# fraunhoferhhi/vvenc

Measured on AMD Instinct MI355X. Metric: frames/sec + bit-exact vs CPU, 1080p/4K 10-bit preset=faster at 1/2/4/8 GPU, higher is better.
Workload: dtype i16; 1 GPU; BASELINE configs[1]: hot-path work lists RECORDED from the reference encoder (1920x1080 10-bit synthetic clip, 65 frames, preset faster; one picture per temporal layer), replayed resident in HBM: a step = one picture's integer-ME SAD windows + sub-pel SATD stages + table calls + fused TU transform/quant lists + DMVR lists on 5 HIP streams; steps follow the GOP's 1:1:2:4:8:16 layer mix from the key; hip_streams=5, sample_pairs_per_frame=175309451, coefficients_per_frame=6951461, recorded_calls_outside_the_lists=0

## Files before the change

### vvenc_amd/csrc/trquant.hip

```cpp
#include "common.h"
#include <stdlib.h>
#include <string.h>
#include <algorithm>
#include <vector>

namespace {

typedef uint32_t u32x2 __attribute__( ( ext_vector_type( 2 ) ) );
typedef uint32_t u32x4 __attribute__( ( ext_vector_type( 4 ) ) );
typedef short    s16x2 __attribute__( ( ext_vector_type( 2 ) ) );

__device__ __forceinline__ int clip3i( int lo, int hi, int v ) { return v < lo ? lo : ( v > hi ? hi : v ); }
__device__ __forceinline__ int sat16( int v ) { return clip3i( -32768, 32767, v ); }
__device__ __forceinline__ int dot2( uint32_t a, uint32_t b, int acc )
{
  return __builtin_amdgcn_sdot2( __builtin_bit_cast( s16x2, a ), __builtin_bit_cast( s16x2, b ), acc, false );
}

struct TrGeom
{
  int w, h, log2w, log2h;
  int skipW, skipH;
  int shift1, shift2;
};
// ... 919 lines not shown
      }
    }
  };
  uint32_t xr[8];
  loadResidual( waveIndex, xr );

  const int rndF1 = A.shF1 > 0 ? 1 << ( A.shF1 - 1 ) : 0, rndF2 = 1 << ( A.shF2 - 1 ), rndI1 = 1 << ( A.shI1 - 1 ), rndI2 = 1 << ( A.shI2 - 1 );
  const bool liveCol = inL < N - A.skipW, liveRow = mxSigma( c32 ) % N < N - A.skipH;
  const v4i zero4 = { 0, 0, 0, 0 };
  sOps[lane]       = liveCol ? *reinterpret_cast<const v4i*>( A.opH->nat[lane] ) : zero4;
  sOps[64 + lane]  = liveRow ? *reinterpret_cast<const v4i*>( A.opV->rowP[lane] ) : zero4;
  const int cP1 = ( liveCol ? A.opH->rowSum[c32] : 0 ) + rndF1, cI1 = A.opV->colSum[c32] + rndI1;
  sInit[c32]      = ( c32 % N < N - A.skipH ? A.opV->rowSum[c32] : 0 ) + rndF2;
  sInit[32 + c32] = A.opH->colSum[c32] + rndI2;
  uint32_t pos[16];
  {
    const u32x4 p0 = *reinterpret_cast<const u32x4*>( A.pos + lane * 16 ), p1 = *reinterpret_cast<const u32x4*>( A.pos + lane * 16 + 8 );
    const uint32_t pw[8] = { p0.x, p0.y, p0.z, p0.w, p1.x, p1.y, p1.z, p1.w };
#pragma unroll
    for( int v = 0; v < 16; v++ ) pos[v] = ( v & 1 ) ? pw[v >> 1] >> 16 : pw[v >> 1] & 0xffffu;
  }
  WAVE_SYNC();
  if( ( A.phaseLimit & 0xff ) == 1 ) return;

  for( int tile = waveIndex; tile < A.tiles; tile += A.waveStride )
  {
    v4i aLo, aHi;
    if( tile != waveIndex ) loadResidual( tile, xr );
#pragma unroll
    for( int g = 0; g < 4; g++ )
    {
      aLo[g] = ( int ) ( __builtin_amdgcn_perm( xr[2 * g + 1], xr[2 * g], 0x06040200u ) ^ 0x80808080u );
      aHi[g] = ( int ) __builtin_amdgcn_perm( xr[2 * g + 1], xr[2 * g], 0x07050301u );
    }
    vvhip_tu_qp qqs[R];
#pragma unroll
    for( int r = 0; r < R; r++ ) { const int tu = tile * TPT + ( blk0 + r ) * TPS + blkL; qqs[r] = tu < A.n ? A.qps[tu] : vvhip_tu_qp{ 32, 0 }; }
    if( ( A.phaseLimit & 0xff ) == 2 ) { int k_ = 0; _Pragma( "unroll" ) for( int g = 0; g < 4; g++ ) k_ ^= aLo[g] ^ aHi[g]; if( k_ == 0x12345678 ) A.stats[0].pad = 1; continue; }

    int d[16];
    v4i bLo, bHi;
    {
      v16i c;
#pragma unroll
      for( int v = 0; v < 16; v++ ) c[v] = cP1;
      const v4i opP1 = sOps[lane];
      MX_PASS( aHi, opP1, aLo, opP1, c, A.shF1 );
      mxSplitSat( d, bLo, bHi );
    }
    {
      v16i c;
#pragma unroll
      for( int g = 0; g < 4; g++ ) { const v4i t = *reinterpret_cast<const v4i*>( &sInit[h * 16 + 4 * g] ); c[4 * g] = t.x; c[4 * g + 1] = t.y; c[4 * g + 2] = t.z; c[4 * g + 3] = t.w; }
      const v4i opP2 = sOps[64 + lane];
      MX_PASS( opP2, bHi, opP2, bLo, c, A.shF2 );
    }
    if( ( A.phaseLimit & 0xff ) == 3 ) { TUMX_KEEP( d ); continue; }

    uint32_t last[R], need[R], big[R];
    bool wide = false, someLevel = false;
#pragma unroll
    for( int r = 0; r < R; r++ )
    {
      const TuMxQ P = tuMxParams( A.q, qqs[r], A.thrVal );
      uint32_t l = 0, mx = 0, bg = 0;
      const int thr4 = P.thres >> 2;
// ... 79 lines not shown
        if( PS == 8 ) { u32x4 v; v.x = rp[0]; v.y = rp[1 % ( PS / 2 )]; v.z = rp[2 % ( PS / 2 )]; v.w = rp[3 % ( PS / 2 )]; *reinterpret_cast<u32x4*>( dst ) = v; } \
        else          { u32x2 v; v.x = rp[0]; v.y = rp[1 % ( PS / 2 )]; *reinterpret_cast<u32x2*>( dst ) = v; } \
      } \
    } \
_Pragma( "unroll" ) \
    for( int r = 0; r < R; r++ ) \
    { \
      const unsigned long long t = vvhipGroupSum64( smallDiff ? ( unsigned long long ) sse32[r] : sse[r], G, lane ); \
      const int tu = tile * TPT + blkL * TPS + blk0 + r; \
      if( A.stats && ( N < 32 || h == 0 ) && inL == r && tu < A.n ) A.stats[tu].sse = t; \
    } }
    const bool allZero = ( N >= TUMX_ZERO_MIN_N ) && __builtin_amdgcn_ballot_w64( someLevel ) == 0ull;
    uint32_t xr2[8];
#define TUMX_REREAD() { _Pragma( "unroll" ) for( int c = 0; c < NP; c++ )                                                                \
      {                                                                                                                                 \
        const int X0 = 16 * h + PS * c;                                                                                                 \
        const int tu = tile * TPT + blkL * TPS + X0 / N;                                                                                \
        const int16_t* src = resi + ( tu < A.n ? A.resiOff[tu] : 0 ) + ( ptrdiff_t ) inL * resiStride + X0 % N;                         \
        if( PS == 8 )                                                                                                                   \
        {                                                                                                                               \
          u32x4 v = { 0, 0, 0, 0 };                                                                                                     \
          if( tu < A.n ) v = reinterpret_cast<const U16*>( src )->v;                                                                    \
          xr2[4 * c] = v.x; xr2[( 4 * c + 1 ) & 7] = v.y; xr2[( 4 * c + 2 ) & 7] = v.z; xr2[( 4 * c + 3 ) & 7] = v.w;                   \
        }                                                                                                                               \
        else                                                                                                                            \
        {                                                                                                                               \
          u32x2 v = { 0, 0 };                                                                                                           \
          if( tu < A.n ) v = reinterpret_cast<const U8*>( src )->v;                                                                     \
          xr2[( 2 * c ) & 7] = v.x; xr2[( 2 * c + 1 ) & 7] = v.y;                                                                       \
        }                                                                                                                               \
      } }
    if( allZero )
    {
#if TUMX_ZERO_KEEP_RESI
#pragma unroll
      for( int k = 0; k < 8; k++ ) xr2[k] = xr[k];
#else
      TUMX_REREAD()
#endif
#pragma unroll
      for( int r = 0; r < R; r++ )
      {
        const int tu = tile * TPT + ( blk0 + r ) * TPS + blkL;
        if( A.stats && ( N < 32 || h == 0 ) && inL == r && tu < A.n )
        {
          int32_t* st = reinterpret_cast<int32_t*>( A.stats + tu );
          st[0] = 0; st[1] = ( int32_t ) last[r]; st[2] = ( int32_t ) need[r]; st[3] = 0;
        }
      }
      if( !( A.phaseLimit & 0x100 ) )
#pragma unroll
      for( int u = 0; u < 16 / PS; u++ )
      {
        const int q = lane + 64 * u, Y = q / ( 32 / PS ), X = PS * ( q % ( 32 / PS ) );
        const int tu = tile * TPT + ( Y / N ) * TPS + X / N;
        if( tu < A.n )
        {
          const size_t at = ( size_t ) tu * N * N + ( Y % N ) * N + X % N;
          if( PS == 8 ) { if( A.level ) *reinterpret_cast<u32x4*>( A.level + at ) = u32x4{ 0, 0, 0, 0 }; if( A.rec ) *reinterpret_cast<u32x4*>( A.rec + at ) = u32x4{ 0, 0, 0, 0 }; }
          else          { if( A.level ) *reinterpret_cast<u32x2*>( A.level + at ) = u32x2{ 0, 0 }; if( A.rec ) *reinterpret_cast<u32x2*>( A.rec + at ) = u32x2{ 0, 0 }; }
        }
      }
#pragma unroll
      for( int v = 0; v < 16; v++ ) d[v] = 0;
      TUMX_TAIL( false )
      continue;
    }
    uint32_t absSum[R];
#define TUMX_LEVELS( MEXPR )                                                                                                           \
    _Pragma( "unroll" ) for( int r = 0; r < R; r++ )                                                                                   \
    {                                                                                                                                  \
      const TuMxQ P = tuMxParams( A.q, qqs[r], A.thrVal );                                                                             \
      uint32_t sum = 0;                                                                                                                \
      const int rsPos = P.rightShift > 0 ? P.rightShift : 0, rndDq = P.rightShift > 0 ? 1 << ( P.rightShift - 1 ) : 0;                \
      const int iscaleL = P.rightShift < 0 ? P.iscale << ( -P.rightShift ) : P.iscale;                                                 \
      _Pragma( "unroll" ) for( int v = r * VPR; v < ( r + 1 ) * VPR; v++ )                                                             \
      {                                                                                                                                \
        const int cv = d[v];                                                                                                           \
        const uint32_t ac = ( uint32_t ) abs( cv );                                                                                    \
        uint32_t m = MEXPR;                                                                                                            \
        m = pos[v] <= last[r] ? m : 0u;                                                                                                \
        sum += m;                                                                                                                      \
        const int sm = cv < 0 ? -( int32_t ) m : ( int32_t ) m;                                                                        \
        const int lv = clip3i( -32768, 32767, sm );                                                                                    \
        stage[( 16 * h + v ) * LP + c32] = ( int16_t ) lv;                                                                             \
        const int cl = med3i( lv, ~P.inMax, P.inMax );                                                                                 \
        const int32_t w_ = ( int32_t ) ( ( uint32_t ) __mul24( cl, iscaleL ) + ( uint32_t ) rndDq ) >> rsPos;    \
        d[v] = clip3i( -32768, 32767, w_ );                                                                                            \
      }                                                                                                                                \
      absSum[r] = sum;                                                                                                                 \
    }
    if( narrow )
    {
#pragma unroll
      for( int r = 0; r < R; r++ )
// ... 83 lines not shown
{
  constexpr int LP = 40;
  struct __attribute__( ( packed, aligned( 2 ) ) ) U16 { u32x4 v; };
  const VvhipTuMx64Ops* __restrict__ O = reinterpret_cast<const VvhipTuMx64Ops*>( A.opH );
  const int lane = threadIdx.x & 63, h = lane >> 5, c32 = lane & 31;
  const v16i zero16 = { 0, 0, 0, 0, 0, 0, 0, 0, 0, 0, 0, 0, 0, 0, 0, 0 };
#define WAVE_SYNC() { __builtin_amdgcn_fence( __ATOMIC_ACQ_REL, "wavefront" ); __builtin_amdgcn_wave_barrier(); }
  const int rndF1 = 1 << ( A.shF1 - 1 ), rndF2 = 1 << ( A.shF2 - 1 ), rndI1 = 1 << ( A.shI1 - 1 ), rndI2 = 1 << ( A.shI2 - 1 );
#pragma unroll
  for( int q = 0; q < 2; q++ )
  {
    sOps[( 0 + q ) * 64 + lane] = *reinterpret_cast<const v4i*>( O->natX[q][lane] );
    sOps[( 2 + q ) * 64 + lane] = *reinterpret_cast<const v4i*>( O->rowPY[q][lane] );
  }
  const int cP1 = O->rowSum[c32] + rndF1;
  const int cI1[2] = { O->colSum[c32] + rndI1, O->colSum[32 + c32] + rndI1 };
  sInit[c32] = O->rowSum[c32] + rndF2;
  sInit[32 + lane] = O->colSum[lane] + rndI2;
  uint32_t pos[16];
  {
    const u32x4 p0 = *reinterpret_cast<const u32x4*>( &O->pos[lane][0] ), p1 = *reinterpret_cast<const u32x4*>( &O->pos[lane][8] );
    const uint32_t pw[8] = { p0.x, p0.y, p0.z, p0.w, p1.x, p1.y, p1.z, p1.w };
#pragma unroll
    for( int v = 0; v < 16; v++ ) pos[v] = ( v & 1 ) ? pw[v >> 1] >> 16 : pw[v >> 1] & 0xffffu;
  }
  WAVE_SYNC();

  for( int tu = waveIndex; tu < A.n; tu += A.waveStride )
  {
    const int16_t* src = resi + A.resiOff[tu];
    const vvhip_tu_qp qq = A.qps[tu];
    int d[16];
    v4i bLo[2], bHi[2];
#pragma unroll
    for( int t = 0; t < 2; t++ )
    {
      v16i acc = zero16;
      v4i aLo[2];
#pragma unroll
      for( int c = 0; c < 2; c++ )
      {
        const int16_t* p = src + ( ptrdiff_t ) ( 32 * t + c32 ) * resiStride + 32 * c + 16 * h;
        const u32x4 x0 = reinterpret_cast<const U16*>( p )->v, x1 = reinterpret_cast<const U16*>( p + 8 )->v;
        const uint32_t xr[8] = { x0.x, x0.y, x0.z, x0.w, x1.x, x1.y, x1.z, x1.w };
        v4i aHi;
#pragma unroll
        for( int g = 0; g < 4; g++ )
        {
          aLo[c][g] = ( int ) ( __builtin_amdgcn_perm( xr[2 * g + 1], xr[2 * g], 0x06040200u ) ^ 0x80808080u );
          aHi[g] = ( int ) __builtin_amdgcn_perm( xr[2 * g + 1], xr[2 * g], 0x07050301u );
        }
        acc = __builtin_amdgcn_mfma_i32_32x32x32_i8( aHi, sOps[c * 64 + lane], acc, 0, 0, 0 );
      }
#pragma unroll
      for( int v = 0; v < 16; v++ ) acc[v] = ( acc[v] << 8 ) + cP1;
#pragma unroll
      for( int c = 0; c < 2; c++ ) acc = __builtin_amdgcn_mfma_i32_32x32x32_i8( aLo[c], sOps[c * 64 + lane], acc, 0, 0, 0 );
#pragma unroll
      for( int v = 0; v < 16; v++ ) d[v] = acc[v] >> A.shF1;
      mxSplitSat( d, bLo[t], bHi[t] );
    }
    {
      v16i acc = zero16;
#pragma unroll
      for( int t = 0; t < 2; t++ ) acc = __builtin_amdgcn_mfma_i32_32x32x32_i8( sOps[( 2 + t ) * 64 + lane], bHi[t], acc, 0, 0, 0 );
#pragma unroll
      for( int g = 0; g < 4; g++ )
      {
        const v4i t4 = *reinterpret_cast<const v4i*>( &sInit[h * 16 + 4 * g] );
        acc[4 * g] = ( acc[4 * g] << 8 ) + t4.x; acc[4 * g + 1] = ( acc[4 * g + 1] << 8 ) + t4.y; acc[4 * g + 2] = ( acc[4 * g + 2] << 8 ) + t4.z; acc[4 * g + 3] = ( acc[4 * g + 3] << 8 ) + t4.w;
      }
#pragma unroll
      for( int t = 0; t < 2; t++ ) acc = __builtin_amdgcn_mfma_i32_32x32x32_i8( sOps[( 2 + t ) * 64 + lane], bLo[t], acc, 0, 0, 0 );
#pragma unroll
      for( int v = 0; v < 16; v++ ) d[v] = acc[v] >> A.shF2;
    }
    const TuMxQ P = tuMxParams( A.q, qq, A.thrVal );
    uint32_t last = 0, mx = 0, big = 0;
    const int thr4 = P.thres >> 2;
#pragma unroll
    for( int v = 0; v < 16; v++ )
    {
      const uint32_t ac = ( uint32_t ) abs( d[v] );
      mx = ac > mx ? ac : mx;
      last = ( ac != 0 && pos[v] > last ) ? pos[v] : last;
      big = ( ( int ) __umul24( ac, ( uint32_t ) P.scale ) > thr4 && pos[v] > big ) ? pos[v] : big;
    }
    { const uint32_t lb = tuMxGroupMaxPk16( last | ( big << 16 ), 64, lane ); last = lb & 0xffffu; big = lb >> 16; }
    mx = vvhipGroupMax32( mx, 64, lane );
    const uint32_t need = ( uint32_t ) ( ( int32_t ) ( ( ( int64_t ) mx * P.scale + P.addN ) >> P.qBits ) != 0 );
    const bool narrow = __builtin_amdgcn_ballot_w64( mx >= 65536u || P.qBits > 30 || P.qBits < 9 ) == 0ull;
    if( !narrow )
    {
      big = 0;
#pragma unroll
      for( int v = 0; v < 16; v++ ) big = ( ( long long ) abs( d[v] ) * ( P.scale << 2 ) > ( long long ) P.thres && pos[v] > big ) ? pos[v] : big;
      big = vvhipGroupMax32( big, 64, lane );
    }
    if( last >= 16 )
    {
      if( big < 16 ) last = 15;
      else if( ( big >> 4 ) != ( last >> 4 ) ) last = ( big >> 4 ) * 16 + 15;
    }
    if( __builtin_amdgcn_ballot_w64( ( ( ( int64_t ) mx * P.scale + P.addQ ) >> P.qBits ) != 0 ) == 0ull )
    {
      if( A.stats && lane == 0 )
      {
        int32_t* st = reinterpret_cast<int32_t*>( A.stats + tu );
        st[0] = 0; st[1] = ( int32_t ) last; st[2] = ( int32_t ) need; st[3] = 0;
      }
      unsigned long long sse0 = 0;
      typedef unsigned short u16x2z __attribute__( ( ext_vector_type( 2 ) ) );
#pragma nounroll
      for( int tc = 0; tc < 4; tc++ )
        {
          const int t = tc >> 1, c = tc & 1;
          const int16_t* p = src + ( ptrdiff_t ) ( 32 * t + c32 ) * resiStride + 32 * c + 16 * h;
          const u32x4 x0 = reinterpret_cast<const U16*>( p )->v, x1 = reinterpret_cast<const U16*>( p + 8 )->v;
          const uint32_t xr[8] = { x0.x, x0.y, x0.z, x0.w, x1.x, x1.y, x1.z, x1.w };
          const u32x4 z4 = { 0, 0, 0, 0 };
          const int q0 = lane + 64 * ( 4 * t + 2 * c );
          const bool dense = !( A.phaseLimit & 0x100 );
          if( A.rec && dense )
          {
            *reinterpret_cast<u32x4*>( A.rec + ( size_t ) tu * 4096 + ( size_t ) q0 * 8 ) = z4;
            *reinterpret_cast<u32x4*>( A.rec + ( size_t ) tu * 4096 + ( size_t ) ( q0 + 64 ) * 8 ) = z4;
          }
          if( A.level && dense )
          {
            *reinterpret_cast<u32x4*>( A.level + ( size_t ) tu * 4096 + ( size_t ) q0 * 8 ) = z4;
            *reinterpret_cast<u32x4*>( A.level + ( size_t ) tu * 4096 + ( size_t ) ( q0 + 64 ) * 8 ) = z4;
          }
          uint32_t magn = 0;
#pragma unroll
          for( int k = 0; k < 8; k++ ) magn |= __builtin_bit_cast( uint32_t, __builtin_bit_cast( u16x2z, xr[k] ) + __builtin_bit_cast( u16x2z, 0x10001000u ) ) & 0xe000e000u;
          if( __builtin_amdgcn_ballot_w64( magn != 0 ) == 0ull )
          {
            uint32_t s32 = 0;
#pragma unroll
            for( int k = 0; k < 8; k++ ) s32 = ( uint32_t ) dot2( xr[k], xr[k], ( int ) s32 );
            sse0 += s32;
          }
          else
#pragma unroll
            for( int k = 0; k < 8; k++ )
            {
              const int e0 = ( int ) ( int16_t ) ( xr[k] & 0xffff ), e1 = ( int ) xr[k] >> 16;
              sse0 += ( unsigned long long ) ( ( long long ) e0 * e0 ) + ( unsigned long long ) ( ( long long ) e1 * e1 );
            }
        }
      sse0 = vvhipGroupSum64( sse0, 64, lane );
      if( A.stats && lane == 0 ) A.stats[tu].sse = sse0;
      continue;
    }
    uint32_t sum = 0;
    {
      const int addP = ( int ) P.addQ, addM = ( int ) ( ( 1u << ( P.qBits & 31 ) ) - 1u ) - addP;
      const int rsPos = P.rightShift > 0 ? P.rightShift : 0, rndDq = P.rightShift > 0 ? 1 << ( P.rightShift - 1 ) : 0;
      const int iscaleL = P.rightShift < 0 ? P.iscale << ( -P.rightShift ) : P.iscale;
#define TU64_LEVEL( SMEXPR )                                                                                                         \
      _Pragma( "unroll" ) for( int v = 0; v < 16; v++ )                                                                                 \
      {                                                                                                                                 \
        const int cv = d[v];                                                                                                            \
        int sm = SMEXPR;                                                                                                                \
        sm = pos[v] <= last ? sm : 0;                                                                                                   \
        sum += ( uint32_t ) abs( sm );                                                                                                  \
        const int lv = clip3i( -32768, 32767, sm );                                                                                     \
        stage[( 16 * h + v ) * LP + c32] = ( int16_t ) lv;                                                                              \
        const int cl = med3i( lv, ~P.inMax, P.inMax );                                                                                  \
        const int32_t w_ = ( int32_t ) ( ( uint32_t ) __mul24( cl, iscaleL ) + ( uint32_t ) rndDq ) >> rsPos;                           \
        d[v] = clip3i( -32768, 32767, w_ );                                                                                             \
      }
      if( narrow ) { TU64_LEVEL( ( __mul24( cv, P.scale ) + ( cv < 0 ? addM : addP ) ) >> P.qBits ) }
      else { TU64_LEVEL( ( cv < 0 ? -( int ) ( ( ( int64_t ) abs( cv ) * P.scale + P.addQ ) >> P.qBits ) : ( int ) ( ( ( int64_t ) abs( cv ) * P.scale + P.addQ ) >> P.qBits ) ) ) }
#undef TU64_LEVEL
    }
    sum = vvhipGroupSum32( sum, 64, lane );
    if( A.stats && lane == 0 )
    {
      int32_t* st = reinterpret_cast<int32_t*>( A.stats + tu );
      st[0] = ( int32_t ) sum; st[1] = ( int32_t ) last; st[2] = ( int32_t ) need; st[3] = 0;
    }
    WAVE_SYNC();
    if( A.level )
#pragma unroll
      for( int u = 0; u < 8; u++ )
      {
        const int q = lane + 64 * u, Y = q >> 3, X = 8 * ( q & 7 );
        u32x4 v = { 0, 0, 0, 0 };
        if( Y < 32 && X < 32 ) v = *reinterpret_cast<const u32x4*>( &stage[Y * LP + X] );
        *reinterpret_cast<u32x4*>( A.level + ( size_t ) tu * 4096 + Y * 64 + X ) = v;
      }
    WAVE_SYNC();
    v4i aLo, aHi;
    mxSplit( d, aLo, aHi );
#pragma unroll
    for( int t = 0; t < 2; t++ )
    {
      v16i c;
#pragma unroll
      for( int v = 0; v < 16; v++ ) c[v] = cI1[t];
      const v4i op = *reinterpret_cast<const v4i*>( O->natTY[t][lane] );
      v16i acc = __builtin_amdgcn_mfma_i32_32x32x32_i8( aHi, op, zero16, 0, 0, 0 );
#pragma unroll
      for( int v = 0; v < 16; v++ ) acc[v] = ( acc[v] << 8 ) + c[v];
      acc = __builtin_amdgcn_mfma_i32_32x32x32_i8( aLo, op, acc, 0, 0, 0 );
#pragma unroll
      for( int v = 0; v < 16; v++ ) d[v] = acc[v] >> A.shI1;
      mxSplitSat( d, bLo[t], bHi[t] );
    }
    unsigned long long sse = 0;
#pragma unroll
    for( int t = 0; t < 2; t++ )
#pragma unroll
      for( int c = 0; c < 2; c++ )
      {
        const int16_t* p = src + ( ptrdiff_t ) ( 32 * t + c32 ) * resiStride + 32 * c + 16 * h;
        const u32x4 x0 = reinterpret_cast<const U16*>( p )->v, x1 = reinterpret_cast<const U16*>( p + 8 )->v;
        const uint32_t xr[8] = { x0.x, x0.y, x0.z, x0.w, x1.x, x1.y, x1.z, x1.w };
        v16i ci;
#pragma unroll
        for( int g = 0; g < 4; g++ ) { const v4i t4 = *reinterpret_cast<const v4i*>( &sInit[32 + 32 * c + h * 16 + 4 * g] ); ci[4 * g] = t4.x; ci[4 * g + 1] = t4.y; ci[4 * g + 2] = t4.z; ci[4 * g + 3] = t4.w; }
        const v4i op = *reinterpret_cast<const v4i*>( O->colPX[c][lane] );
        v16i acc = __builtin_amdgcn_mfma_i32_32x32x32_i8( op, bHi[t], zero16, 0, 0, 0 );
#pragma unroll
        for( int v = 0; v < 16; v++ ) acc[v] = ( acc[v] << 8 ) + ci[v];
        acc = __builtin_amdgcn_mfma_i32_32x32x32_i8( op, bLo[t], acc, 0, 0, 0 );
        typedef unsigned short u16x2t __attribute__( ( ext_vector_type( 2 ) ) );
        uint32_t rp[8], magn = 0;
#pragma unroll
        for( int k = 0; k < 8; k++ )
        {
          rp[k] = __builtin_bit_cast( uint32_t, __builtin_amdgcn_cvt_pk_i16( acc[2 * k] >> A.shI2, acc[2 * k + 1] >> A.shI2 ) );
          magn |= __builtin_bit_cast( uint32_t, __builtin_bit_cast( u16x2t, rp[k] ) + __builtin_bit_cast( u16x2t, 0x10001000u ) ) & 0xe000e000u;
          magn |= __builtin_bit_cast( uint32_t, __builtin_bit_cast( u16x2t, xr[k] ) + __builtin_bit_cast( u16x2t, 0x10001000u ) ) & 0xe000e000u;
        }
        if( __builtin_amdgcn_ballot_w64( magn != 0 ) == 0ull )
        {
          uint32_t s32 = 0;
#pragma unroll
          for( int k = 0; k < 8; k++ )
          {
            const uint32_t df = __builtin_bit_cast( uint32_t, __builtin_bit_cast( s16x2, xr[k] ) - __builtin_bit_cast( s16x2, rp[k] ) );
            s32 = ( uint32_t ) dot2( df, df, ( int ) s32 );
          }
          sse += s32;
        }
        else
#pragma unroll
          for( int k = 0; k < 8; k++ )
          {
            const int e0 = ( int ) ( int16_t ) ( xr[k] & 0xffff ) - ( int ) ( int16_t ) ( rp[k] & 0xffff ), e1 = ( ( int ) xr[k] >> 16 ) - ( ( int ) rp[k] >> 16 );
            sse += ( unsigned long long ) ( ( long long ) e0 * e0 ) + ( unsigned long long ) ( ( long long ) e1 * e1 );
          }
        if( A.rec )
        {
          int16_t* dst = A.rec + ( size_t ) tu * 4096 + ( 32 * t + c32 ) * 64 + 32 * c + 16 * h;
          u32x4 a, b; a.x = rp[0]; a.y = rp[1]; a.z = rp[2]; a.w = rp[3]; b.x = rp[4]; b.y = rp[5]; b.z = rp[6]; b.w = rp[7];
          *reinterpret_cast<u32x4*>( dst ) = a; *reinterpret_cast<u32x4*>( dst + 8 ) = b;
        }
      }
    sse = vvhipGroupSum64( sse, 64, lane );
    if( A.stats && lane == 0 ) A.stats[tu].sse = sse;
  }
#undef WAVE_SYNC
}

__device__ __forceinline__ void tuMxPairSync( uint32_t* ctr, uint32_t& gen, int lane )
{
  __builtin_amdgcn_fence( __ATOMIC_RELEASE, "workgroup" );
  if( lane == 0 ) atomicAdd( ctr, 1u );
  gen += 2;
  while( *reinterpret_cast<volatile uint32_t*>( ctr ) < gen ) __builtin_amdgcn_s_sleep( 1 );
  __builtin_amdgcn_fence( __ATOMIC_ACQUIRE, "workgroup" );
}

__device__ __forceinline__ void
tuMx64PairBody( int16_t* __restrict__ stage, int32_t* __restrict__ sInit , v4i* __restrict__ sOps , int32_t* __restrict__ xch ,
                uint32_t* __restrict__ ctr, const int p , const int pairIndex, const int pairStride,
                const int16_t* __restrict__ resi, const int resiStride, const TuMxArgs& A )
{
  constexpr int LP = 40, XP = 17;
  struct __attribute__( ( packed, aligned( 2 ) ) ) U16 { u32x4 v; };
  const VvhipTuMx64Ops* __restrict__ O = reinterpret_cast<const VvhipTuMx64Ops*>( A.opH );
  const int lane = threadIdx.x & 63, h = lane >> 5, c32 = lane & 31;
  const v16i zero16 = { 0, 0, 0, 0, 0, 0, 0, 0, 0, 0, 0, 0, 0, 0, 0, 0 };
#define WAVE_SYNC() { __builtin_amdgcn_fence( __ATOMIC_ACQ_REL, "wavefront" ); __builtin_amdgcn_wave_barrier(); }
  const int rndF1 = 1 << ( A.shF1 - 1 ), rndF2 = 1 << ( A.shF2 - 1 ), rndI1 = 1 << ( A.shI1 - 1 ), rndI2 = 1 << ( A.shI2 - 1 );
#pragma unroll
  for( int q = 0; q < 2; q++ )
// ... 154 lines not shown
      const v4i op = sOps[( 6 + c ) * 64 + lane];
      const v16i lo = __builtin_amdgcn_mfma_i32_32x32x32_i8( op, bLo, ci, 0, 0, 0 );
      const v16i hi = __builtin_amdgcn_mfma_i32_32x32x32_i8( op, bHi, zero16, 0, 0, 0 );
      uint32_t rp[8];
#pragma unroll
      for( int k = 0; k < 8; k++ )
      {
        const int v0 = ( ( hi[2 * k] << 8 ) + lo[2 * k] ) >> A.shI2, v1 = ( ( hi[2 * k + 1] << 8 ) + lo[2 * k + 1] ) >> A.shI2;
        rp[k] = __builtin_bit_cast( uint32_t, __builtin_amdgcn_cvt_pk_i16( v0, v1 ) );
        const int e0 = ( int ) ( int16_t ) ( xr[k] & 0xffff ) - ( int ) ( int16_t ) ( rp[k] & 0xffff ), e1 = ( ( int ) xr[k] >> 16 ) - ( ( int ) rp[k] >> 16 );
        sse += ( unsigned long long ) ( ( long long ) e0 * e0 ) + ( unsigned long long ) ( ( long long ) e1 * e1 );
      }
      if( A.rec )
      {
        int16_t* dst = A.rec + ( size_t ) tu * 4096 + ( 32 * p + c32 ) * 64 + 32 * c + 16 * h;
        u32x4 a, b; a.x = rp[0]; a.y = rp[1]; a.z = rp[2]; a.w = rp[3]; b.x = rp[4]; b.y = rp[5]; b.z = rp[6]; b.w = rp[7];
        *reinterpret_cast<u32x4*>( dst ) = a; *reinterpret_cast<u32x4*>( dst + 8 ) = b;
      }
    }
    sse = vvhipGroupSum64( sse, 64, lane );
    if( lane == 0 ) { xMine[16] = ( int32_t ) ( uint32_t ) sse; xMine[XP + 16] = ( int32_t ) ( uint32_t ) ( sse >> 32 ); }
    tuMxPairSync( ctr, gen, lane );
    if( A.stats && p == 0 && lane == 0 )
    {
      const unsigned long long o = ( unsigned long long ) ( uint32_t ) xOther[16] | ( ( unsigned long long ) ( uint32_t ) xOther[XP + 16] << 32 );
      A.stats[tu].sse = sse + o;
    }
  }
#undef WAVE_SYNC
}

struct TuMxJobs { int nJobs; int pair64; int waveStart[8]; int size[8]; TuMxArgs j[8]; };

template<int KIND>
__global__ void __launch_bounds__( 256, KIND == 3 ? 2 : 3 )
tuMxMultiKernel( const int16_t* __restrict__ resi, int resiStride, TuMxJobs jobs )
{
  constexpr bool WITH4 = KIND >= 1, WITH64 = KIND >= 2, PAIR64 = KIND == 3;
  __shared__ __attribute__( ( aligned( 16 ) ) ) int16_t stage[4][32 * 40];
  __shared__ __attribute__( ( aligned( 16 ) ) ) int32_t sInit[4][WITH64 ? 96 : 64];
  __shared__ v4i sOps[4][PAIR64 ? 512 : ( WITH64 ? 256 : 128 )];
  __shared__ int32_t xch[PAIR64 ? 2 : 1][PAIR64 ? 2 * 64 * 17 : 1];
  __shared__ uint32_t pairCtr[2];
  if( PAIR64 ) { if( threadIdx.x < 2 ) pairCtr[threadIdx.x] = 0; __syncthreads(); }
  const int wv = __builtin_amdgcn_readfirstlane( ( int ) ( threadIdx.x >> 6 ) );
  const int wave = blockIdx.x * 4 + wv;
  int k = 0;
#pragma unroll
  for( int i = 1; i < 8; i++ ) if( i < jobs.nJobs && wave >= jobs.waveStart[i] ) k = i;
  const int w = wave - jobs.waveStart[k];
  if( w >= jobs.j[k].waveStride ) return;
  const int rs = jobs.j[k].resiStride ? jobs.j[k].resiStride : resiStride;
  if( jobs.size[k] == 32 )      tuMxBody<32>( stage[wv], sInit[wv], sOps[wv], w, resi, rs, jobs.j[k] );
  else if( jobs.size[k] == 16 ) tuMxBody<16>( stage[wv], sInit[wv], sOps[wv], w, resi, rs, jobs.j[k] );
  else if( jobs.size[k] == 8 )  tuMxBody<8>( stage[wv], sInit[wv], sOps[wv], w, resi, rs, jobs.j[k] );
  else if( WITH4 && jobs.size[k] == 4 )   tuMxBody<4>( stage[wv], sInit[wv], sOps[wv], w, resi, rs, jobs.j[k] );
  else if( WITH64 && jobs.size[k] == 64 )
  {
    if( PAIR64 ) tuMx64PairBody( stage[wv], sInit[wv], sOps[wv], xch[wv >> 1], &pairCtr[wv >> 1], w & 1, w >> 1, jobs.j[k].waveStride >> 1, resi, rs, jobs.j[k] );
    else         tuMx64Body( stage[wv], sInit[wv], sOps[wv], w, resi, rs, jobs.j[k] );
  }
}

__global__ void __launch_bounds__( 256 )
dequantCoreKernel( int maxX, int maxY, int scale, const int16_t* __restrict__ q, size_t qStride, int32_t* __restrict__ coef, int rightShift, int inMax, int32_t trMax )
{
  const int w = maxX + 1, total = w * ( maxY + 1 );
  for( int n = blockIdx.x * blockDim.x + threadIdx.x; n < total; n += gridDim.x * blockDim.x )
  {
    const int y = n / w, x = n - y * w;
    const int c = clip3i( -( inMax + 1 ), inMax, ( int ) q[x + y * qStride] );
    int32_t v;
    if( rightShift > 0 ) v = ( int32_t ) ( ( uint32_t ) ( c * scale ) + ( 1u << ( rightShift - 1 ) ) ) >> rightShift;
    else                 v = ( int32_t ) ( ( uint32_t ) ( c * scale ) << ( -rightShift ) );
    coef[n] = clip3i( -( trMax + 1 ), trMax, v );
  }
}

__global__ void __launch_bounds__( 256 )
// ... 393 lines not shown
        mj.j[nJobs] = ra;
      }
      nJobs++;
    }
    if( mx )
    {
      TuMxJobs xj; xj.nJobs = nJobs; xj.pair64 = pair64 ? 1 : 0;
      long waves = 0;
      for( int i = 0; i < nJobs; i++ )
      {
        const vvhip_tu_job& jb = jobs[order[first + i]];
        const TuRowArgs& ra = rowArgs[i];
        TuMxArgs& xa = xj.j[i];
        const int z = ra.gf.log2w - 2, tpt = jb.width == 64 ? 1 : ( 32 / jb.width ) * ( 32 / jb.width );
        xa.resiOff = jb.d_resi_off; xa.n = jb.n;
        xa.shF1 = ra.gf.shift1; xa.shF2 = ra.gf.shift2; xa.shI1 = ra.gi.shift1; xa.shI2 = ra.gi.shift2; xa.skipW = ra.gf.skipW; xa.skipH = ra.gf.skipH;
        xa.q = ra.q;
        xa.opH = ctx->d_tuMx + jb.tr_hor * 4 + z; xa.opV = ctx->d_tuMx + jb.tr_ver * 4 + z; xa.pos = ctx->d_tuMxPos + z * 64 * 16;
        if( jb.width == 64 ) { xa.opH = reinterpret_cast<const VvhipTuMxOps*>( ctx->d_tuMx64 ); xa.opV = xa.opH; xa.pos = nullptr; }
        xa.qps = jb.d_qp; xa.thrVal = jb.thr_val; xa.level = jb.d_level; xa.rec = jb.d_rec_resi; xa.stats = jb.d_stats;
        xa.tiles = ( jb.n + tpt - 1 ) / tpt; xa.phaseLimit = tuPhaseLimit() | ( ctx->tuSparse ? 0x100 : 0 );
        const int repeat = budget ? repeatOf( first + i ) : tuRepeat();
        xa.waveStride = wavesPer( first + i ) * ( ( xa.tiles + repeat - 1 ) / repeat );
        xa.resiStride = strides ? strides[order[first + i]] : 0;
        if( wavesPer( first + i ) == 2 ) waves = ( waves + 1 ) & ~1l;
        xj.waveStart[i] = ( int ) waves; xj.size[i] = jb.width;
        waves += xa.waveStride;
      }
      for( int i = nJobs; i < 8; i++ ) { xj.waveStart[i] = 0x7fffffff; xj.size[i] = 0; }
      bool any4 = false;
      for( int i = 0; i < xj.nJobs; i++ ) any4 |= xj.size[i] == 4 || xj.size[i] == 64;
      bool any64 = false;
      for( int i = 0; i < xj.nJobs; i++ ) any64 |= xj.size[i] == 64;
      const dim3 grid( ( unsigned ) ( ( waves + 3 ) / 4 ) );
      static const int ldsPad = getenv( "VVHIP_TU_LDS_PAD" ) ? atoi( getenv( "VVHIP_TU_LDS_PAD" ) ) : 0;
      static bool padSet = false;
      if( ldsPad > 0 && !padSet )
      {
        padSet = true;
        ( void ) hipFuncSetAttribute( ( const void* ) tuMxMultiKernel<0>, hipFuncAttributeMaxDynamicSharedMemorySize, ldsPad );
        ( void ) hipFuncSetAttribute( ( const void* ) tuMxMultiKernel<1>, hipFuncAttributeMaxDynamicSharedMemorySize, ldsPad );
        ( void ) hipFuncSetAttribute( ( const void* ) tuMxMultiKernel<2>, hipFuncAttributeMaxDynamicSharedMemorySize, ldsPad );
        ( void ) hipFuncSetAttribute( ( const void* ) tuMxMultiKernel<3>, hipFuncAttributeMaxDynamicSharedMemorySize, ldsPad );
      }
      if( any64 && pair64 ) hipLaunchKernelGGL( tuMxMultiKernel<3>, grid, dim3( 256 ), ldsPad, ctx->stream, d_resi, resi_stride, xj );
      else if( any64 ) hipLaunchKernelGGL( tuMxMultiKernel<2>, grid, dim3( 256 ), ldsPad, ctx->stream, d_resi, resi_stride, xj );
      else if( any4 ) hipLaunchKernelGGL( tuMxMultiKernel<1>, grid, dim3( 256 ), ldsPad, ctx->stream, d_resi, resi_stride, xj );
      else            hipLaunchKernelGGL( tuMxMultiKernel<0>, grid, dim3( 256 ), ldsPad, ctx->stream, d_resi, resi_stride, xj );
    }
    else
    {
      mj.nJobs = nJobs;
      for( int i = nJobs; i < 4; i++ ) { mj.blockStart[i] = 0x7fffffff; mj.size[i] = 0; }
      hipLaunchKernelGGL( tuRdoRowMultiKernel, dim3( ( unsigned ) blocks ), dim3( 256 ), 0, ctx->stream, d_resi, resi_stride, mj );
    }
    VVHIP_LAUNCH_CHECK( ctx );
  }
  return VVHIP_OK;
}

static bool trSizeOk( int n ) { return n == 4 || n == 8 || n == 16 || n == 32 || n == 64; }

int vvhip_fast_fwd_core( vvhip_ctx* ctx, int tr_size, const int16_t* d_tc, const int32_t* d_src, int32_t* d_dst, unsigned line, unsigned reduced_line, unsigned cutoff, int shift )
{
  if( !ctx ) return VVHIP_E_ARG;
  if( !trSizeOk( tr_size ) || !d_tc || !d_src || !d_dst || reduced_line > line || cutoff > ( unsigned ) tr_size || line > 64 || shift < 1 || shift > 31 )
    return vvhip_fail( ctx, VVHIP_E_ARG, "vvhip_fast_fwd_core: trSize %d line %u/%u cutoff %u shift %d", tr_size, reduced_line, line, cutoff, shift );
  const unsigned total = reduced_line * cutoff;
  if( !total ) return VVHIP_OK;
  hipLaunchKernelGGL( fastFwdCoreKernel, dim3( ( total + 255 ) / 256 ), dim3( 256 ), 0, ctx->stream, tr_size, d_tc, d_src, d_dst, line, reduced_line, cutoff, shift );
  VVHIP_LAUNCH_CHECK( ctx );
  return VVHIP_OK;
}

int vvhip_fast_inv_core( vvhip_ctx* ctx, int tr_size, const int16_t* d_it, const int32_t* d_src, int32_t* d_dst, unsigned lines, unsigned reduced_lines, unsigned rows )
{
  if( !ctx ) return VVHIP_E_ARG;
  if( !trSizeOk( tr_size ) || !d_it || !d_src || !d_dst || reduced_lines > lines || rows > ( unsigned ) tr_size || lines > 64 )
    return vvhip_fail( ctx, VVHIP_E_ARG, "vvhip_fast_inv_core: trSize %d lines %u/%u rows %u", tr_size, reduced_lines, lines, rows );
  const unsigned total = reduced_lines * tr_size;
  if( !total ) return VVHIP_OK;
// ... 98 lines not shown
```

Baseline: 14500 frames/s.

## Compute residual energy early to skip all-zero TU reread; launch single-wave workgroups

Residual energy and a small-magnitude flag are computed from the already-loaded residual registers before the transform. All-zero TUs then store SSE directly instead of rereading the residual, and the 64x64 path hoists its zero stores into one flat loop and only rereads when magnitudes are large. The multi-job TU kernel gains a waves-per-block template parameter and by default launches 64-thread workgroups, except for the paired-64 form, to reduce LDS per block and improve scheduling. The energy math runs on every tile, adding some ALU work to non-zero TUs, and the default launch shape changes.

```diff
diff --git a/vvenc_amd/csrc/trquant.hip b/vvenc_amd/csrc/trquant.hip
--- a/vvenc_amd/csrc/trquant.hip
+++ b/vvenc_amd/csrc/trquant.hip
@@ -975,6 +975,23 @@
     {
       aLo[g] = ( int ) ( __builtin_amdgcn_perm( xr[2 * g + 1], xr[2 * g], 0x06040200u ) ^ 0x80808080u );
       aHi[g] = ( int ) __builtin_amdgcn_perm( xr[2 * g + 1], xr[2 * g], 0x07050301u );
+    }
+    int eng[R];
+    bool smallResi = false;
+    if( N >= TUMX_ZERO_MIN_N )
+    {
+      typedef unsigned short u16x2e __attribute__( ( ext_vector_type( 2 ) ) );
+      uint32_t magn = 0;
+#pragma unroll
+      for( int r = 0; r < R; r++ ) eng[r] = 0;
+#pragma unroll
+      for( int k = 0; k < 8; k++ )
+      {
+        const int slot = ( PS * ( k / ( PS / 2 ) ) ) / N < R ? ( PS * ( k / ( PS / 2 ) ) ) / N : 0;
+        eng[slot] = dot2( xr[k], xr[k], eng[slot] );
+        magn |= __builtin_bit_cast( uint32_t, __builtin_bit_cast( u16x2e, xr[k] ) + __builtin_bit_cast( u16x2e, 0x10001000u ) ) & 0xe000e000u;
+      }
+      smallResi = __builtin_amdgcn_ballot_w64( magn != 0 ) == 0ull;
     }
     vvhip_tu_qp qqs[R];
 #pragma unroll
@@ -1120,12 +1137,6 @@
       } }
     if( allZero )
     {
-#if TUMX_ZERO_KEEP_RESI
-#pragma unroll
-      for( int k = 0; k < 8; k++ ) xr2[k] = xr[k];
-#else
-      TUMX_REREAD()
-#endif
 #pragma unroll
       for( int r = 0; r < R; r++ )
       {
@@ -1149,6 +1160,18 @@
           else          { if( A.level ) *reinterpret_cast<u32x2*>( A.level + at ) = u32x2{ 0, 0 }; if( A.rec ) *reinterpret_cast<u32x2*>( A.rec + at ) = u32x2{ 0, 0 }; }
         }
       }
+      if( smallResi )
+      {
+#pragma unroll
+        for( int r = 0; r < R; r++ )
+        {
+          const unsigned long long t = vvhipGroupSum64( ( unsigned long long ) ( uint32_t ) eng[r], G, lane );
+          const int tu = tile * TPT + blkL * TPS + blk0 + r;
+          if( A.stats && ( N < 32 || h == 0 ) && inL == r && tu < A.n ) A.stats[tu].sse = t;
+        }
+        continue;
+      }
+      TUMX_REREAD()
 #pragma unroll
       for( int v = 0; v < 16; v++ ) d[v] = 0;
       TUMX_TAIL( false )
@@ -1298,6 +1321,9 @@
     const vvhip_tu_qp qq = A.qps[tu];
     int d[16];
     v4i bLo[2], bHi[2];
+    typedef unsigned short u16x2z __attribute__( ( ext_vector_type( 2 ) ) );
+    int eng = 0;
+    uint32_t magn = 0;
 #pragma unroll
     for( int t = 0; t < 2; t++ )
     {
@@ -1316,6 +1342,12 @@
           aLo[c][g] = ( int ) ( __builtin_amdgcn_perm( xr[2 * g + 1], xr[2 * g], 0x06040200u ) ^ 0x80808080u );
           aHi[g] = ( int ) __builtin_amdgcn_perm( xr[2 * g + 1], xr[2 * g], 0x07050301u );
         }
+#pragma unroll
+        for( int k = 0; k < 8; k++ )
+        {
+          eng = dot2( xr[k], xr[k], eng );
+          magn |= __builtin_bit_cast( uint32_t, __builtin_bit_cast( u16x2z, xr[k] ) + __builtin_bit_cast( u16x2z, 0x10001000u ) ) & 0xe000e000u;
+        }
         acc = __builtin_amdgcn_mfma_i32_32x32x32_i8( aHi, sOps[c * 64 + lane], acc, 0, 0, 0 );
       }
 #pragma unroll
@@ -1375,46 +1407,39 @@
         int32_t* st = reinterpret_cast<int32_t*>( A.stats + tu );
         st[0] = 0; st[1] = ( int32_t ) last; st[2] = ( int32_t ) need; st[3] = 0;
       }
-      unsigned long long sse0 = 0;
-      typedef unsigned short u16x2z __attribute__( ( ext_vector_type( 2 ) ) );
+      if( !( A.phaseLimit & 0x100 ) )
+      {
+        char* zr = reinterpret_cast<char*>( A.rec + ( size_t ) tu * 4096 );
+        char* zl = reinterpret_cast<char*>( A.level + ( size_t ) tu * 4096 );
+        uint32_t zo = ( uint32_t ) lane * 16u;
+        asm volatile( "" : "+v"( zo ) );
+        const u32x4 z4 = { 0, 0, 0, 0 };
+#pragma unroll
+        for( int u = 0; u < 8; u++ )
+        {
+          if( A.rec ) *reinterpret_cast<u32x4*>( zr + ( zo + 1024u * u ) ) = z4;
+          if( A.level ) *reinterpret_cast<u32x4*>( zl + ( zo + 1024u * u ) ) = z4;
+        }
+      }
+      unsigned long long sse0 = ( unsigned long long ) ( uint32_t ) eng;
+      if( __builtin_amdgcn_ballot_w64( magn != 0 ) != 0ull )
+      {
+        sse0 = 0;
 #pragma nounroll
-      for( int tc = 0; tc < 4; tc++ )
+        for( int tc = 0; tc < 4; tc++ )
         {
           const int t = tc >> 1, c = tc & 1;
           const int16_t* p = src + ( ptrdiff_t ) ( 32 * t + c32 ) * resiStride + 32 * c + 16 * h;
           const u32x4 x0 = reinterpret_cast<const U16*>( p )->v, x1 = reinterpret_cast<const U16*>( p + 8 )->v;
           const uint32_t xr[8] = { x0.x, x0.y, x0.z, x0.w, x1.x, x1.y, x1.z, x1.w };
-          const u32x4 z4 = { 0, 0, 0, 0 };
-          const int q0 = lane + 64 * ( 4 * t + 2 * c );
-          const bool dense = !( A.phaseLimit & 0x100 );
-          if( A.rec && dense )
+#pragma unroll
+          for( int k = 0; k < 8; k++ )
           {
-            *reinterpret_cast<u32x4*>( A.rec + ( size_t ) tu * 4096 + ( size_t ) q0 * 8 ) = z4;
-            *reinterpret_cast<u32x4*>( A.rec + ( size_t ) tu * 4096 + ( size_t ) ( q0 + 64 ) * 8 ) = z4;
+            const int e0 = ( int ) ( int16_t ) ( xr[k] & 0xffff ), e1 = ( int ) xr[k] >> 16;
+            sse0 += ( unsigned long long ) ( ( long long ) e0 * e0 ) + ( unsigned long long ) ( ( long long ) e1 * e1 );
           }
-          if( A.level && dense )
-          {
-            *reinterpret_cast<u32x4*>( A.level + ( size_t ) tu * 4096 + ( size_t ) q0 * 8 ) = z4;
-            *reinterpret_cast<u32x4*>( A.level + ( size_t ) tu * 4096 + ( size_t ) ( q0 + 64 ) * 8 ) = z4;
-          }
-          uint32_t magn = 0;
-#pragma unroll
-          for( int k = 0; k < 8; k++ ) magn |= __builtin_bit_cast( uint32_t, __builtin_bit_cast( u16x2z, xr[k] ) + __builtin_bit_cast( u16x2z, 0x10001000u ) ) & 0xe000e000u;
-          if( __builtin_amdgcn_ballot_w64( magn != 0 ) == 0ull )
-          {
-            uint32_t s32 = 0;
-#pragma unroll
-            for( int k = 0; k < 8; k++ ) s32 = ( uint32_t ) dot2( xr[k], xr[k], ( int ) s32 );
-            sse0 += s32;
-          }
-          else
-#pragma unroll
-            for( int k = 0; k < 8; k++ )
-            {
-              const int e0 = ( int ) ( int16_t ) ( xr[k] & 0xffff ), e1 = ( int ) xr[k] >> 16;
-              sse0 += ( unsigned long long ) ( ( long long ) e0 * e0 ) + ( unsigned long long ) ( ( long long ) e1 * e1 );
-            }
         }
+      }
       sse0 = vvhipGroupSum64( sse0, 64, lane );
       if( A.stats && lane == 0 ) A.stats[tu].sse = sse0;
       continue;
@@ -1448,11 +1473,14 @@
       st[0] = ( int32_t ) sum; st[1] = ( int32_t ) last; st[2] = ( int32_t ) need; st[3] = 0;
     }
     WAVE_SYNC();
+    int laneL = lane;
+    asm volatile( "" : "+v"( laneL ) );
+    const int hL = laneL >> 5, c32L = laneL & 31;
     if( A.level )
 #pragma unroll
       for( int u = 0; u < 8; u++ )
       {
-        const int q = lane + 64 * u, Y = q >> 3, X = 8 * ( q & 7 );
+        const int q = laneL + 64 * u, Y = q >> 3, X = 8 * ( q & 7 );
         u32x4 v = { 0, 0, 0, 0 };
         if( Y < 32 && X < 32 ) v = *reinterpret_cast<const u32x4*>( &stage[Y * LP + X] );
         *reinterpret_cast<u32x4*>( A.level + ( size_t ) tu * 4096 + Y * 64 + X ) = v;
@@ -1466,7 +1494,7 @@
       v16i c;
 #pragma unroll
       for( int v = 0; v < 16; v++ ) c[v] = cI1[t];
-      const v4i op = *reinterpret_cast<const v4i*>( O->natTY[t][lane] );
+      const v4i op = *reinterpret_cast<const v4i*>( O->natTY[t][laneL] );
       v16i acc = __builtin_amdgcn_mfma_i32_32x32x32_i8( aHi, op, zero16, 0, 0, 0 );
 #pragma unroll
       for( int v = 0; v < 16; v++ ) acc[v] = ( acc[v] << 8 ) + c[v];
@@ -1477,17 +1505,17 @@
     }
     unsigned long long sse = 0;
 #pragma unroll
-    for( int t = 0; t < 2; t++ )
-#pragma unroll
-      for( int c = 0; c < 2; c++ )
+    for( int c = 0; c < 2; c++ )
+#pragma unroll
+      for( int t = 0; t < 2; t++ )
       {
         const int16_t* p = src + ( ptrdiff_t ) ( 32 * t + c32 ) * resiStride + 32 * c + 16 * h;
         const u32x4 x0 = reinterpret_cast<const U16*>( p )->v, x1 = reinterpret_cast<const U16*>( p + 8 )->v;
         const uint32_t xr[8] = { x0.x, x0.y, x0.z, x0.w, x1.x, x1.y, x1.z, x1.w };
         v16i ci;
 #pragma unroll
-        for( int g = 0; g < 4; g++ ) { const v4i t4 = *reinterpret_cast<const v4i*>( &sInit[32 + 32 * c + h * 16 + 4 * g] ); ci[4 * g] = t4.x; ci[4 * g + 1] = t4.y; ci[4 * g + 2] = t4.z; ci[4 * g + 3] = t4.w; }
-        const v4i op = *reinterpret_cast<const v4i*>( O->colPX[c][lane] );
+        for( int g = 0; g < 4; g++ ) { const v4i t4 = *reinterpret_cast<const v4i*>( &sInit[32 + 32 * c + hL * 16 + 4 * g] ); ci[4 * g] = t4.x; ci[4 * g + 1] = t4.y; ci[4 * g + 2] = t4.z; ci[4 * g + 3] = t4.w; }
+        const v4i op = *reinterpret_cast<const v4i*>( O->colPX[c][laneL] );
         v16i acc = __builtin_amdgcn_mfma_i32_32x32x32_i8( op, bHi[t], zero16, 0, 0, 0 );
 #pragma unroll
         for( int v = 0; v < 16; v++ ) acc[v] = ( acc[v] << 8 ) + ci[v];
@@ -1521,7 +1549,7 @@
           }
         if( A.rec )
         {
-          int16_t* dst = A.rec + ( size_t ) tu * 4096 + ( 32 * t + c32 ) * 64 + 32 * c + 16 * h;
+          int16_t* dst = A.rec + ( size_t ) tu * 4096 + ( 32 * t + c32L ) * 64 + 32 * c + 16 * hL;
           u32x4 a, b; a.x = rp[0]; a.y = rp[1]; a.z = rp[2]; a.w = rp[3]; b.x = rp[4]; b.y = rp[5]; b.z = rp[6]; b.w = rp[7];
           *reinterpret_cast<u32x4*>( dst ) = a; *reinterpret_cast<u32x4*>( dst + 8 ) = b;
         }
@@ -1742,19 +1770,20 @@
 
 struct TuMxJobs { int nJobs; int pair64; int waveStart[8]; int size[8]; TuMxArgs j[8]; };
 
-template<int KIND>
-__global__ void __launch_bounds__( 256, KIND == 3 ? 2 : 3 )
+template<int KIND, int WPB>
+__global__ void __launch_bounds__( 64 * WPB, KIND == 3 ? 2 : 3 )
 tuMxMultiKernel( const int16_t* __restrict__ resi, int resiStride, TuMxJobs jobs )
 {
   constexpr bool WITH4 = KIND >= 1, WITH64 = KIND >= 2, PAIR64 = KIND == 3;
-  __shared__ __attribute__( ( aligned( 16 ) ) ) int16_t stage[4][32 * 40];
-  __shared__ __attribute__( ( aligned( 16 ) ) ) int32_t sInit[4][WITH64 ? 96 : 64];
-  __shared__ v4i sOps[4][PAIR64 ? 512 : ( WITH64 ? 256 : 128 )];
+  static_assert( WPB == 4 || ( WPB == 1 && !PAIR64 ), "the pair form needs both waves of a pair in one workgroup" );
+  __shared__ __attribute__( ( aligned( 16 ) ) ) int16_t stage[WPB][32 * 40];
+  __shared__ __attribute__( ( aligned( 16 ) ) ) int32_t sInit[WPB][WITH64 ? 96 : 64];
+  __shared__ v4i sOps[WPB][PAIR64 ? 512 : ( WITH64 ? 256 : 128 )];
   __shared__ int32_t xch[PAIR64 ? 2 : 1][PAIR64 ? 2 * 64 * 17 : 1];
   __shared__ uint32_t pairCtr[2];
   if( PAIR64 ) { if( threadIdx.x < 2 ) pairCtr[threadIdx.x] = 0; __syncthreads(); }
-  const int wv = __builtin_amdgcn_readfirstlane( ( int ) ( threadIdx.x >> 6 ) );
-  const int wave = blockIdx.x * 4 + wv;
+  const int wv = WPB == 1 ? 0 : __builtin_amdgcn_readfirstlane( ( int ) ( threadIdx.x >> 6 ) );
+  const int wave = blockIdx.x * WPB + wv;
   int k = 0;
 #pragma unroll
   for( int i = 1; i < 8; i++ ) if( i < jobs.nJobs && wave >= jobs.waveStart[i] ) k = i;
@@ -2214,21 +2243,32 @@
       for( int i = 0; i < xj.nJobs; i++ ) any4 |= xj.size[i] == 4 || xj.size[i] == 64;
       bool any64 = false;
       for( int i = 0; i < xj.nJobs; i++ ) any64 |= xj.size[i] == 64;
-      const dim3 grid( ( unsigned ) ( ( waves + 3 ) / 4 ) );
+      const char* wg1Env = getenv( "VVHIP_TU_WG1" );
+      const int wpb = ( ( !wg1Env || atoi( wg1Env ) != 0 ) && !( any64 && pair64 ) ) ? 1 : 4;
+      const dim3 grid( ( unsigned ) ( ( waves + wpb - 1 ) / wpb ) );
       static const int ldsPad = getenv( "VVHIP_TU_LDS_PAD" ) ? atoi( getenv( "VVHIP_TU_LDS_PAD" ) ) : 0;
       static bool padSet = false;
       if( ldsPad > 0 && !padSet )
       {
         padSet = true;
-        ( void ) hipFuncSetAttribute( ( const void* ) tuMxMultiKernel<0>, hipFuncAttributeMaxDynamicSharedMemorySize, ldsPad );
-        ( void ) hipFuncSetAttribute( ( const void* ) tuMxMultiKernel<1>, hipFuncAttributeMaxDynamicSharedMemorySize, ldsPad );
-        ( void ) hipFuncSetAttribute( ( const void* ) tuMxMultiKernel<2>, hipFuncAttributeMaxDynamicSharedMemorySize, ldsPad );
-        ( void ) hipFuncSetAttribute( ( const void* ) tuMxMultiKernel<3>, hipFuncAttributeMaxDynamicSharedMemorySize, ldsPad );
-      }
-      if( any64 && pair64 ) hipLaunchKernelGGL( tuMxMultiKernel<3>, grid, dim3( 256 ), ldsPad, ctx->stream, d_resi, resi_stride, xj );
-      else if( any64 ) hipLaunchKernelGGL( tuMxMultiKernel<2>, grid, dim3( 256 ), ldsPad, ctx->stream, d_resi, resi_stride, xj );
-      else if( any4 ) hipLaunchKernelGGL( tuMxMultiKernel<1>, grid, dim3( 256 ), ldsPad, ctx->stream, d_resi, resi_stride, xj );
-      else            hipLaunchKernelGGL( tuMxMultiKernel<0>, grid, dim3( 256 ), ldsPad, ctx->stream, d_resi, resi_stride, xj );
+        ( void ) hipFuncSetAttribute( ( const void* ) tuMxMultiKernel<0, 4>, hipFuncAttributeMaxDynamicSharedMemorySize, ldsPad );
+        ( void ) hipFuncSetAttribute( ( const void* ) tuMxMultiKernel<1, 4>, hipFuncAttributeMaxDynamicSharedMemorySize, ldsPad );
+        ( void ) hipFuncSetAttribute( ( const void* ) tuMxMultiKernel<2, 4>, hipFuncAttributeMaxDynamicSharedMemorySize, ldsPad );
+        ( void ) hipFuncSetAttribute( ( const void* ) tuMxMultiKernel<3, 4>, hipFuncAttributeMaxDynamicSharedMemorySize, ldsPad );
+        ( void ) hipFuncSetAttribute( ( const void* ) tuMxMultiKernel<0, 1>, hipFuncAttributeMaxDynamicSharedMemorySize, ldsPad );
+        ( void ) hipFuncSetAttribute( ( const void* ) tuMxMultiKernel<1, 1>, hipFuncAttributeMaxDynamicSharedMemorySize, ldsPad );
+        ( void ) hipFuncSetAttribute( ( const void* ) tuMxMultiKernel<2, 1>, hipFuncAttributeMaxDynamicSharedMemorySize, ldsPad );
+      }
+      if( any64 && pair64 ) hipLaunchKernelGGL( ( tuMxMultiKernel<3, 4> ), grid, dim3( 256 ), ldsPad, ctx->stream, d_resi, resi_stride, xj );
+      else if( wpb == 1 )
+      {
+        if( any64 )     hipLaunchKernelGGL( ( tuMxMultiKernel<2, 1> ), grid, dim3( 64 ), ldsPad, ctx->stream, d_resi, resi_stride, xj );
+        else if( any4 ) hipLaunchKernelGGL( ( tuMxMultiKernel<1, 1> ), grid, dim3( 64 ), ldsPad, ctx->stream, d_resi, resi_stride, xj );
+        else            hipLaunchKernelGGL( ( tuMxMultiKernel<0, 1> ), grid, dim3( 64 ), ldsPad, ctx->stream, d_resi, resi_stride, xj );
+      }
+      else if( any64 ) hipLaunchKernelGGL( ( tuMxMultiKernel<2, 4> ), grid, dim3( 256 ), ldsPad, ctx->stream, d_resi, resi_stride, xj );
+      else if( any4 ) hipLaunchKernelGGL( ( tuMxMultiKernel<1, 4> ), grid, dim3( 256 ), ldsPad, ctx->stream, d_resi, resi_stride, xj );
+      else            hipLaunchKernelGGL( ( tuMxMultiKernel<0, 4> ), grid, dim3( 256 ), ldsPad, ctx->stream, d_resi, resi_stride, xj );
     }
     else
     {
```

Measured after the change: 15290 frames/s, median of 6. +5.5%, better.
